# massquantity/LibRecommender

Hardware: AMD Instinct MI355X
Metric: train samples/sec (higher is better)
Workload: dtype f32 (split-bf16 x6 MFMA products, f32 accumulate); 1 GPU; DeepFM ranking train step, 1M users x 1M items x 200 sparse fields (10,000,200 sparse rows), embed_size=64, hidden=(128,64,32), Zipf(1.05) ids; per_gpu_batch=16384, global_batch=16384, fields=202, embed_size=64, table_rows=12000202, parallelism=single, launch=one hipGraph replay per step

## Files before the change

### include/libreco_hip.h

```cpp
#ifndef LIBRECO_HIP_H_
#define LIBRECO_HIP_H_

#include <stddef.h>
#include <stdint.h>

#ifdef __cplusplus
extern "C" {
#endif

#define LR_OK 0
#define LR_EINVAL (-1)
#define LR_ESHAPE (-2)
#define LR_EWORKSPACE (-3)

typedef void* lr_stream_t;

const char* lr_strerror(int code);
int lr_abi_version(void);
int lr_graph_foreign_nodes(void* graph, int* n_nodes_out);

int lr_embed_gather_f32(const float* table, int64_t V, int K, const int32_t* idx,
                        int64_t n, float* out, lr_stream_t stream);

#define LR_COMBINER_SUM 0
// ... 219 lines not shown
int lr_adam_coef_store(lr_adam_hp hp, void* coef_dev, lr_stream_t stream);
int lr_adam_dense_dc_f32(float* table, float* m, float* v, int64_t n, const float* grad,
                         const void* coef_dev, lr_stream_t stream);
int lr_fm_rows_adam_dc_f32(float* table, float* m, float* v, float* lin, float* lin_m, float* lin_v,
                           int64_t V, int K, const float* ge, const float* gl, const float* wp,
                           const float* bn_a, const float* bn_c, const float* lin_scale, int64_t B,
                           int F, const int32_t* seg_pos, const int32_t* seg_rows,
                           const int32_t* seg_start, const int32_t* n_seg, const void* coef_dev,
                           void* ws, size_t ws_bytes, lr_stream_t stream);
int lr_embed_scatter_adam_dc_f32(float* table, float* m, float* v, int64_t V, int K, const float* grad,
                                 const int32_t* seg_pos, const int32_t* seg_rows, const int32_t* seg_start,
                                 const int32_t* n_seg, int64_t n_max, const void* coef_dev,
                                 void* ws, size_t ws_bytes, lr_stream_t stream);
int lr_embed_scatter_adam_lin_dc_f32(float* table, float* m, float* v, int64_t V, int K, const float* grad,
                                     float* lin, float* lin_m, float* lin_v, const float* glin,
                                     const int32_t* seg_pos, const int32_t* seg_rows,
                                     const int32_t* seg_start, const int32_t* n_seg, int64_t n_max,
                                     const void* coef_dev, lr_stream_t stream);

int lr_table_colstats_f32(const float* table, int64_t V, int K, const int32_t* idx, int64_t B, int F, int C,
                          float* partial, lr_stream_t stream);
int lr_bn_remainder_f32(float* G, const float* x, const float* a, const float* c, int64_t rows,
                        int64_t rows_per_plane, int64_t period, int Kp, lr_stream_t stream);

size_t lr_segments_fields_ws_bytes(int64_t B, int F);
int lr_segments_build_fields(const int32_t* idxT, int64_t B, int F, const int32_t* field_row_start,
                             int32_t* seg_pos, int32_t* seg_rows, int32_t* seg_start,
                             int32_t* n_seg, int32_t* slotT, void* ws, size_t ws_bytes,
                             lr_stream_t stream);
int lr_segments_build_fields_runs(const int32_t* idxT, int64_t B, int F, const int32_t* field_row_start,
                                  int32_t* seg_pos, int32_t* seg_rows, int32_t* seg_start,
                                  int32_t* n_seg, int32_t* slotT, int32_t* runT, void* ws, size_t ws_bytes,
                                  lr_stream_t stream);

size_t lr_owner_partition_ws_bytes(int64_t n_max, int W);
int lr_owner_partition_i32(const int32_t* rows, const int32_t* n_seg, int64_t n_max, int W, int32_t* perm,
                           int32_t* send_ids, int64_t* counts, void* ws, size_t ws_bytes, lr_stream_t stream);

size_t lr_din_attn_ws_bytes(int64_t B, int L, int K, int H);
int lr_din_attn_path(int K, int L, int backward);
int lr_din_build_ids_i32(const int32_t* users, const int32_t* items, const int32_t* sparse, int sparse_ld,
                         const int32_t* cols, int n_plain, const int32_t* seqs, const int32_t* lens, int64_t B, int L,
                         int32_t user_off, int32_t item_off, int32_t sparse_off, int32_t* ids, lr_stream_t stream);
int lr_din_attn_pool_fwd_f32(const float* item_table, int64_t V, int K,
                             const int32_t* item, const int32_t* seq, const int32_t* len,
                             int64_t B, int L, const float* W1, const float* b1,
                             const float* W2, const float* b2, int H, float* out,
                             float* attn, float* hid , int32_t* order_out ,
                             lr_stream_t stream);
int lr_din_attn_pool_bwd_f32(const float* item_table, int64_t V, int K,
                             const int32_t* item, const int32_t* seq, const int32_t* len,
                             int64_t B, int L, const float* W1, const float* b1,
                             const float* W2, const float* b2, int H, const float* attn,
                             const float* gout, float* gq, float* gkey, float* gW1,
                             float* gb1, float* gW2, float* gb2, void* ws, size_t ws_bytes,
                             lr_stream_t stream);
int lr_din_attn_pool_bwd_parts_f32(const float* item_table, int64_t V, int K,
                                   const int32_t* item, const int32_t* seq, const int32_t* len,
                                   int64_t B, int L, const float* W1, const float* b1,
                                   const float* W2, const float* b2, int H, const float* attn,
                                   const float* gout, float* gq, float* gkey, float* gW1,
                                   float* gb1, float* gW2, float* gb2, void* ws, size_t ws_bytes,
                                   int parts, int keep_pad_rows, const float* hid ,
                                   const int32_t* order , lr_stream_t stream);
int lr_din_attn_dense_fwd_f32(const float* q, const float* keys, int K, const int32_t* len,
                              int64_t B, int L, const float* W1, const float* b1,
// ... 365 lines not shown
```

### librecommender_amd/_lib.py

```python
from __future__ import annotations

import ctypes as C
import os
from pathlib import Path

LIB_PATH = Path(__file__).resolve().parent / "lib" / "liblibreco_hip.so"

LR_OK, LR_EINVAL, LR_ESHAPE, LR_EWORKSPACE = 0, -1, -2, -3
ABI_VERSION = 26

COMBINERS = {"sum": 0, "mean": 1, "sqrtn": 2}


class AdamHP(C.Structure):

    _fields_ = [
        ("lr", C.c_double),
        ("beta1", C.c_double),
        ("beta2", C.c_double),
        ("eps", C.c_double),
        ("weight_decay", C.c_double),
        ("step", C.c_int32),
        ("tf_style", C.c_int32),
    ]
# ... 102 lines not shown
    "lr_bitmap_ids_i32": (_int, [_p, _i64, _i64, _p, _int, _p]),
    "lr_row_slots_i32": (_int, [_p, _p, _i64, _p, _int, _p]),
    "lr_spmm_csr_adam_f32": (_int, [_p, _p, _p, _i64, _i64, _p, _int, _p, _p, _p, _p, _p, _p, _f32, AdamHP, _p, _sz, _int, _p]),
    "lr_din_build_ids_i32": (_int, [_p, _p, _p, _int, _p, _int, _p, _p, _i64, _int, _int, _int, _int, _p, _p]),
    "lr_softmax_ce_supported": (_int, [_i64, _i64, _int]),
    "lr_softmax_ce_fwd_ws_bytes": (_sz, [_i64, _i64, _int, _int]),
    "lr_softmax_ce_fwd_f32": (_int, [_p, _i64, _p, _i64, _int, _p, _p, _p, _i64, _p, _p, _p, _p, _sz, _int, _p]),
    "lr_softmax_ce_bwd_cols_f32": (_int, [_p, _i64, _p, _i64, _int, _p, _p, _p, _i64, _p, _p, _p, _int, _p]),
    "lr_reduce_job_bytes": (_sz, []),
    "lr_reduce_partials_multi_f32": (_int, [_p, _int, _i64, _p]),
    "lr_pair_mlp_supported": (_int, [_int, _int]),
    "lr_pair_mlp_f32": (_int, [_p, _i64, _p, _i64, _int, _p, _p, _int, _p, _f32, _p, _i64, _int, _p]),
    "lr_pair_mlp_sb_f32": (_int, [_p, _i64, _p, _i64, _int, _p, _p, _int, _p, _f32, _p, _i64, _int, _p]),
    "lr_score_topk_test_mute": (None, [_int]),
    "lr_mfma_f32_probe": (_int, [_int, _int, _p, _p]),
    "lr_probe_occupy": (_int, [_int, _sz, _i64, _p]),
    "lr_clock_probe": (_int, [_p, _p]),
    "lr_clock_probe_slots": (_int, []),
    "lr_mlp_tail3_resident_blocks": (_int, []),
    "lr_adam_coef_bytes": (_sz, []),
    "lr_adam_coef_store": (_int, [AdamHP, _p, _p]),
    "lr_adam_dense_dc_f32": (_int, [_p, _p, _p, _i64, _p, _p, _p]),
    "lr_fm_rows_adam_dc_f32": (_int, [_p, _p, _p, _p, _p, _p, _i64, _int, _p, _p, _p, _p, _p, _p, _i64,
                                      _int, _p, _p, _p, _p, _p, _p, _sz, _p]),
    "lr_embed_scatter_adam_dc_f32": (_int, [_p, _p, _p, _i64, _int, _p, _p, _p, _p, _p, _i64, _p, _p, _sz, _p]),
    "lr_embed_scatter_adam_lin_dc_f32": (_int, [_p, _p, _p, _i64, _int, _p, _p, _p, _p, _p, _p, _p, _p, _p, _i64, _p, _p]),
    "lr_table_colstats_f32": (_int, [_p, _i64, _int, _p, _i64, _int, _int, _p, _p]),
    "lr_bn_remainder_f32": (_int, [_p, _p, _p, _p, _i64, _i64, _i64, _int, _p]),
    "lr_csr_laplacian_ws_bytes": (_sz, [_i64]),
    "lr_csr_laplacian_build": (_int, [_p, _p, _i64, _i64, _i64, _p, _p, _p, _p, _p, _p, _sz, _p]),
    "lr_segments_fields_ws_bytes": (_sz, [_i64, _int]),
    "lr_segments_build_fields": (_int, [_p, _i64, _int, _p, _p, _p, _p, _p, _p, _p, _sz, _p]),
    "lr_segments_build_fields_runs": (_int, [_p, _i64, _int, _p, _p, _p, _p, _p, _p, _p, _p, _sz, _p]),
    "lr_owner_partition_ws_bytes": (_sz, [_i64, _int]),
    "lr_owner_partition_i32": (_int, [_p, _p, _i64, _int, _p, _p, _p, _p, _sz, _p]),
    "lr_din_attn_ws_bytes": (_sz, [_i64, _int, _int, _int]),
    "lr_din_attn_path": (_int, [_int, _int, _int]),
    "lr_din_attn_pool_fwd_f32": (_int, [_p, _i64, _int, _p, _p, _p, _i64, _int, _p, _p, _p, _p,
                                        _int, _p, _p, _p, _p, _p]),
    "lr_din_attn_pool_bwd_f32": (_int, [_p, _i64, _int, _p, _p, _p, _i64, _int, _p, _p, _p, _p,
                                        _int, _p, _p, _p, _p, _p, _p, _p, _p, _p, _sz, _p]),
    "lr_din_attn_pool_bwd_parts_f32": (_int, [_p, _i64, _int, _p, _p, _p, _i64, _int, _p, _p, _p, _p,
                                              _int, _p, _p, _p, _p, _p, _p, _p, _p, _p, _sz, _int, _int, _p, _p, _p]),
    "lr_din_attn_dense_fwd_f32": (_int, [_p, _p, _int, _p, _i64, _int, _p, _p, _p, _p, _int, _p,
                                         _p, _p]),
    "lr_din_attn_dense_bwd_f32": (_int, [_p, _p, _int, _p, _i64, _int, _p, _p, _p, _p, _int, _p,
                                         _p, _p, _p, _p, _p, _p, _p, _p, _sz, _p]),
    "lr_score_topk_ws_bytes": (_sz, [_i64, _i64, _int, _int]),
    "lr_score_topk_f32": (_int, [_p, _i64, _p, _i64, _int, _p, _p, _p, _int, _i64, _p, _p, _p,
                                 _sz, _p]),
    "lr_score_topk_sb_f32": (_int, [_p, _i64, _p, _i64, _int, _p, _p, _p, _int, _i64, _p, _p, _p,
                                 _sz, _p]),
    "lr_score_topk_filter_kp": (_int, [_int]),
    "lr_score_topk_filter_ws_bytes": (_sz, [_i64, _i64, _int, _int]),
    "lr_score_topk_filter_f32": (_int, [_p, _i64, _p, _i64, _int, _p, _p, _p, _int, _i64, _p, _p, _p,
                                        _sz, _int, _int, _p, _p]),
    "lr_topk_merge_f32": (_int, [_p, _p, _int, _i64, _int, _p, _p, _p]),
    "lr_ivf_supported": (_int, [_i64, _i64, _int, _int, _int, _int]),
    "lr_ivf_search_ws_bytes": (_sz, [_i64, _i64, _int, _int, _int, _int]),
    "lr_ivf_build_ws_bytes": (_sz, [_i64, _int]),
    "lr_ivf_centroids_ws_bytes": (_sz, [_i64, _int]),
    "lr_ivf_assign_f32": (_int, [_p, _i64, _p, _int, _int, _p, _p, _p]),
    "lr_ivf_build_lists": (_int, [_p, _i64, _int, _p, _p, _p, _sz, _p]),
    "lr_ivf_centroids_f32": (_int, [_p, _i64, _int, _p, _p, _i64, _int, _p, _p, _sz, _p]),
    "lr_ivf_search_f32": (_int, [_p, _i64, _p, _int, _p, _p, _p, _i64, _int, _p, _p, _p, _int, _int, _p, _p, _p, _sz, _p]),
    "lr_ivf_sq8_supported": (_int, [_i64, _i64, _int, _int, _int, _int, _int]),
# ... 175 lines not shown
```

### librecommender_amd/csrc/segments.hip

```cpp
#include <cstring>

#include <rocprim/rocprim.hpp>

#include "common.hpp"

namespace lr {

__global__ __launch_bounds__(kBlock) void seg_keys_kernel(const int32_t* __restrict__ idx,
                                                          int64_t n, uint32_t V,
                                                          uint32_t* __restrict__ keys) {
  const int64_t stride = static_cast<int64_t>(gridDim.x) * kBlock;
  for (int64_t i = static_cast<int64_t>(blockIdx.x) * kBlock + threadIdx.x; i < n; i += stride) {
    const int32_t id = idx[i];
    keys[i] = (id >= 0 && static_cast<uint32_t>(id) < V) ? static_cast<uint32_t>(id) : V;
  }
}

__global__ __launch_bounds__(kBlock) void seg_heads_kernel(const uint32_t* __restrict__ keys,
                                                           int64_t n, uint32_t V,
                                                           int32_t* __restrict__ heads,
                                                           int32_t* __restrict__ n_seg,
                                                           int32_t* __restrict__ seg_start) {
  const int64_t stride = static_cast<int64_t>(gridDim.x) * kBlock;
  const int64_t t0 = static_cast<int64_t>(blockIdx.x) * kBlock + threadIdx.x;
// ... 150 lines not shown
#pragma unroll
    for (int s = 0; s < kFSE; ++s) x[s] = buf[wid * kFSW + s * 64 + lane];
  }
  if (n_pass == 0) {
#pragma unroll
    for (int s = 0; s < kFSE; ++s) buf[wid * kFSW + s * 64 + lane] = x[s];
  }
  __syncthreads();

  int nv = 0, nh = 0;
  uint64_t* dst = sorted + static_cast<int64_t>(f) * B;
#pragma unroll
  for (int s = 0; s < kFSE; ++s) {
    const int i = wid * kFSW + s * 64 + lane;
    const uint32_t key = static_cast<uint32_t>(x[s] >> 32);
    const bool valid = key != kKeyInvalid;
    const bool head = valid && (i == 0 || static_cast<uint32_t>(buf[i > 0 ? i - 1 : 0] >> 32) != key);
    nv += __popcll(__ballot(valid));
    nh += __popcll(__ballot(head));
    if (i < B) dst[i] = x[s];
  }
  __syncthreads();
  if (lane == 0) { wsum[wid * 2] = nv; wsum[wid * 2 + 1] = nh; }
  __syncthreads();
  if (tid == 0) {
    int tv = 0, th = 0;
    for (int w = 0; w < kSortWaves; ++w) { tv += wsum[2 * w]; th += wsum[2 * w + 1]; }
    fcount[2 * f] = tv;
    fcount[2 * f + 1] = th;
  }
}

constexpr int kEmitThreads = 1024;
constexpr int kEmitWaves = kEmitThreads / 64;

__global__ __launch_bounds__(kEmitThreads) void seg_field_emit_kernel(
    const uint64_t* __restrict__ sorted, const int32_t* __restrict__ fcount, int B, int F,
    const int32_t* __restrict__ frs, int32_t* __restrict__ seg_pos, int32_t* __restrict__ seg_rows,
    int32_t* __restrict__ seg_start, int32_t* __restrict__ n_seg, int32_t* __restrict__ slotT,
    int32_t* __restrict__ runT) {
  __shared__ int red[2][kEmitWaves];
  __shared__ int wh[kEmitWaves];
  const int f = blockIdx.x;
  const int tid = threadIdx.x, wid = tid >> 6, lane = tid & 63;
  const uint64_t lt = (1ull << lane) - 1ull;
  int bv = 0, bh = 0;
  for (int g = tid; g < f; g += kEmitThreads) { bv += fcount[2 * g]; bh += fcount[2 * g + 1]; }
#pragma unroll
  for (int o = 32; o > 0; o >>= 1) { bv += __shfl_xor(bv, o); bh += __shfl_xor(bh, o); }
  if (lane == 0) { red[0][wid] = bv; red[1][wid] = bh; }
  __syncthreads();
  int base_v = 0, base_h = 0;
#pragma unroll
  for (int w = 0; w < kEmitWaves; ++w) { base_v += red[0][w]; base_h += red[1][w]; }
  const int nv = fcount[2 * f];
  const int32_t lo = frs[f];
  const uint64_t* src = sorted + static_cast<int64_t>(f) * B;
  const int chunk = ((B + kEmitWaves - 1) / kEmitWaves + 63) / 64 * 64;
  const int i0 = wid * chunk, i1 = (i0 + chunk) < B ? (i0 + chunk) : B;
  auto is_head = [&](int i, uint32_t key) {
    return i < nv && (i == 0 || static_cast<uint32_t>(src[i - 1] >> 32) != key);
  };
  int heads = 0;
  for (int i = i0 + lane; i < i0 + chunk; i += 64) {
    const bool h = i < i1 && is_head(i, static_cast<uint32_t>(src[i < B ? i : 0] >> 32));
    heads += __popcll(__ballot(h));
  }
  if (lane == 0) wh[wid] = heads;
  __syncthreads();
  int run = base_h;
  for (int w = 0; w < wid; ++w) run += wh[w];
  for (int i = i0 + lane; i < i0 + chunk; i += 64) {
    const bool in = i < i1;
    const uint64_t e = src[in ? i : 0];
    const uint32_t key = static_cast<uint32_t>(e >> 32);
    const int p = static_cast<int>(static_cast<uint32_t>(e));
    const bool h = in && is_head(i, key);
    const uint64_t hb = __ballot(h);
    if (in) {
      const bool valid = i < nv;
      if (valid) seg_pos[base_v + i] = p * F + f;
      if (slotT != nullptr) slotT[static_cast<int64_t>(f) * B + p] = valid ? base_v + i : -1;
      if (runT != nullptr) runT[static_cast<int64_t>(f) * B + p] = valid ? run + __popcll(hb & (lt | (1ull << lane))) - 1 : -1;
      if (h) {
        const int r = run + __popcll(hb & lt);
        seg_rows[r] = lo + static_cast<int32_t>(key);
        seg_start[r] = base_v + i;
      }
    }
    run += __popcll(hb);
  }
  if (f == F - 1 && tid == 0) {
    const int tot_h = base_h + fcount[2 * f + 1];
    seg_start[tot_h] = base_v + nv;
    n_seg[0] = tot_h;
  }
}

constexpr int kRsKPT = 8;
constexpr int kRsKPB = kBlock * kRsKPT;
constexpr int kRsWaves = kBlock / 64;
constexpr int kRsKPW = kRsKPB / kRsWaves;
constexpr int64_t kRsMaxN = int64_t(1) << 22;

__global__ __launch_bounds__(kBlock) void rs_hist_kernel(const uint32_t* __restrict__ keys, int64_t n, int shift, int nblk,
                                                         int32_t* __restrict__ hist) {
  __shared__ int cnt[256];
  const int tid = threadIdx.x;
  cnt[tid] = 0;
  __syncthreads();
  const int64_t base = static_cast<int64_t>(blockIdx.x) * kRsKPB;
#pragma unroll
  for (int st = 0; st < kRsKPT; ++st) {
    const int64_t i = base + st * kBlock + tid;
    if (i < n) atomicAdd(&cnt[(keys[i] >> shift) & 255u], 1);
  }
  __syncthreads();
  hist[static_cast<int64_t>(tid) * nblk + blockIdx.x] = cnt[tid];
}

__global__ __launch_bounds__(64) void rs_scan_kernel(int32_t* __restrict__ hist, int nblk, int32_t* __restrict__ tot) {
  const int d = blockIdx.x, lane = threadIdx.x;
  int32_t* row = hist + static_cast<int64_t>(d) * nblk;
  int carry = 0;
  for (int b0 = 0; b0 < nblk; b0 += 64) {
    const int b = b0 + lane;
    const int v = b < nblk ? row[b] : 0;
    int x = v;
#pragma unroll
    for (int o = 1; o < 64; o <<= 1) {
      const int y = __shfl_up(x, o);
// ... 135 lines not shown
    rocprim::counting_iterator<int32_t> iota(0);
    e = rocprim::radix_sort_pairs(nullptr, need, w.keys_in, w.keys_out, iota, seg_pos, static_cast<size_t>(n), 0u,
                                  static_cast<unsigned>(bits), s);
    if (e != hipSuccess) return static_cast<int>(e);
    if (need > w.prim_bytes) return LR_EWORKSPACE;
    e = rocprim::radix_sort_pairs(w.prim, need, w.keys_in, w.keys_out, iota, seg_pos, static_cast<size_t>(n), 0u,
                                  static_cast<unsigned>(bits), s);
    if (e != hipSuccess) return static_cast<int>(e);
  }

  hipLaunchKernelGGL(seg_heads_kernel, dim3(grid), dim3(kBlock), 0, s, w.keys_out, n, Vu,
                     w.rank, n_seg, seg_start);
  need = 0;
  e = rocprim::inclusive_scan(nullptr, need, w.rank, w.rank, static_cast<size_t>(n),
                              rocprim::plus<int32_t>(), s);
  if (e != hipSuccess) return static_cast<int>(e);
  if (need > w.prim_bytes) return LR_EWORKSPACE;
  e = rocprim::inclusive_scan(w.prim, need, w.rank, w.rank, static_cast<size_t>(n),
                              rocprim::plus<int32_t>(), s);
  if (e != hipSuccess) return static_cast<int>(e);

  hipLaunchKernelGGL(seg_emit_kernel, dim3(grid), dim3(kBlock), 0, s, w.keys_out, w.rank, n,
                     Vu, seg_pos, seg_rows, seg_start, n_seg, pos_to_seg);
  return launch_status();
}

extern "C" size_t lr_segments_fields_ws_bytes(int64_t B, int F) {
  if (B < 0 || F < 1) return 0;
  return align_up(static_cast<size_t>(B) * F * 8) + align_up(static_cast<size_t>(F) * 8);
}

static int build_fields_impl(const int32_t* idxT, int64_t B, int F, const int32_t* field_row_start, int32_t* seg_pos,
                             int32_t* seg_rows, int32_t* seg_start, int32_t* n_seg, int32_t* slotT, int32_t* runT, void* ws,
                             size_t ws_bytes, lr_stream_t stream) {
  LR_CHECK_ARG(B >= 1 && F >= 1);
  LR_CHECK_ARG(idxT && field_row_start && seg_pos && seg_rows && seg_start && n_seg && ws);
  if (B > kFS || B * F >= (int64_t(1) << 31)) return LR_ESHAPE;
  if (ws_bytes < lr_segments_fields_ws_bytes(B, F)) return LR_EWORKSPACE;
  hipStream_t s = as_stream(stream);
  uint64_t* sorted = static_cast<uint64_t*>(ws);
  int32_t* fcount = reinterpret_cast<int32_t*>(static_cast<char*>(ws) + align_up(static_cast<size_t>(B) * F * 8));
  const size_t lds = static_cast<size_t>(kFS) * 8 + kSortWaves * 256 * 4 + kSortWaves * 2 * 4;
  static bool attr_set = false;
  if (!attr_set) {
    hipError_t e = hipFuncSetAttribute(reinterpret_cast<const void*>(seg_field_sort_kernel),
                                       hipFuncAttributeMaxDynamicSharedMemorySize, static_cast<int>(lds));
    if (e != hipSuccess) return static_cast<int>(e);
    attr_set = true;
  }
  hipLaunchKernelGGL(seg_field_sort_kernel, dim3(F), dim3(kSortThreads), lds, s, idxT, static_cast<int>(B),
                     field_row_start, sorted, fcount);
  hipLaunchKernelGGL(seg_field_emit_kernel, dim3(F), dim3(kEmitThreads), 0, s, sorted, fcount,
                     static_cast<int>(B), F, field_row_start, seg_pos, seg_rows, seg_start, n_seg, slotT, runT);
  return launch_status();
}

extern "C" int lr_segments_build_fields(const int32_t* idxT, int64_t B, int F, const int32_t* field_row_start,
                                        int32_t* seg_pos, int32_t* seg_rows, int32_t* seg_start, int32_t* n_seg,
                                        int32_t* slotT, void* ws, size_t ws_bytes, lr_stream_t stream) {
  return build_fields_impl(idxT, B, F, field_row_start, seg_pos, seg_rows, seg_start, n_seg, slotT, nullptr, ws, ws_bytes,
                           stream);
}

extern "C" int lr_segments_build_fields_runs(const int32_t* idxT, int64_t B, int F, const int32_t* field_row_start,
                                             int32_t* seg_pos, int32_t* seg_rows, int32_t* seg_start, int32_t* n_seg,
                                             int32_t* slotT, int32_t* runT, void* ws, size_t ws_bytes, lr_stream_t stream) {
  LR_CHECK_ARG(runT != nullptr);
  return build_fields_impl(idxT, B, F, field_row_start, seg_pos, seg_rows, seg_start, n_seg, slotT, runT, ws, ws_bytes,
                           stream);
}

constexpr int kOwnChunk = 1024;
constexpr int kOwnMaxW = 64;

template <bool kPlace>
__device__ __forceinline__ void owner_chunk(const int32_t* __restrict__ rows, int n, int W, int chunk, int (*cnt)[4][kOwnMaxW],
                                            int* my_owner, int* my_rank) {
  const int tid = threadIdx.x, wid = tid >> 6, lane = tid & 63;
  const uint64_t lt = (1ull << lane) - 1ull;
#pragma unroll
  for (int it = 0; it < 4; ++it) {
    const int i = chunk * kOwnChunk + it * kBlock + tid;
    const int o = i < n ? static_cast<int>(static_cast<uint32_t>(rows[i]) % static_cast<uint32_t>(W)) : -1;
    int rank = 0;
    for (int w = 0; w < W; ++w) {
      const uint64_t mk = __ballot(o == w);
      if (o == w) rank = __popcll(mk & lt);
      if (lane == 0) cnt[it][wid][w] = __popcll(mk);
    }
    if (kPlace) { my_owner[it] = o; my_rank[it] = rank; }
  }
}

__global__ __launch_bounds__(kBlock) void owner_count_kernel(const int32_t* __restrict__ rows, const int32_t* __restrict__ n_seg,
// ... 110 lines not shown
```

### librecommender_amd/layers/dense.py

```python
from __future__ import annotations

import math
import os
from typing import List, Optional, Sequence

import torch
import torch.nn.functional as F

from .. import _lib, ops


class DenseParams:

    def __init__(self, device: torch.device, seed: int = 42):
        self.device = device
        self.gen = torch.Generator(device=device)
        self.gen.manual_seed(seed + 1)
        self._specs = []
        self.params = {}
        self.flat = self.grad = self.m = self.v = None

    def add(self, name: str, shape: Sequence[int], init: str) -> str:
        assert self.flat is None, "finalize() already called"
        self._specs.append((name, tuple(shape), init))
# ... 343 lines not shown
    dgamma = (XhG * W).sum(1)
    dbeta = W @ sgz
    s = gamma * inv
    c = s * inv * (dgamma / B)
    a = s * (dbeta / B) - c * mean
    io.bn_a, io.bn_c = a.contiguous(), c.contiguous()
    return dgamma, dbeta, dW, sgz


class FoldedL1Kernels:

    STAT_CHUNKS = 8

    def __init__(self, P, bn, layer, F: int, K: int, device, stat_chunks: Optional[int] = None):
        self.P, self.bn, self.layer, self.F, self.K, self.device = P, bn, layer, int(F), int(K), device
        n, H1 = self.F * self.K, P[layer.w].shape[1]
        f32 = dict(dtype=torch.float32, device=device)
        self.H1 = H1
        if stat_chunks is not None:
            self.STAT_CHUNKS = int(stat_chunks)
        self.stat_partial = torch.empty((self.F, self.STAT_CHUNKS, 2, self.K), **f32)
        self.mean, self.inv, self.s, self.t = (torch.empty(n, **f32) for _ in range(4))
        self.n_slabs = _lib.load().lr_deepfm_l1_fold_bias_slabs(n)
        self.bias_partial = torch.empty((self.n_slabs, H1), **f32)
        self.bp = torch.empty(H1, **f32)
        self.bn_ac = torch.empty(2 * n, **f32)
        self.bn_a, self.bn_c = self.bn_ac[:n], self.bn_ac[n:]

    @staticmethod
    def supported(H1: int) -> bool:
        return H1 in (64, 128, 256)

    def forward(self, io: "FusedL1IO", seg, field_row_start, B: int, cache_slots: Optional[torch.Tensor] = None,
                sync=None) -> torch.Tensor:
        P, bn, l0, st = self.P, self.bn, self.layer, ops._stream()
        W, b = P[l0.w], P[l0.b]
        n = self.F * self.K
        if bn is not None:
            if seg is None:
                ops.table_colstats(io.table, io.idx, self.STAT_CHUNKS, out=self.stat_partial)
            elif cache_slots is None:
                ops._call("lr_fm_field_stats_f32", ops._ptr(io.table), self.K, ops._ptr(seg.rows), ops._ptr(seg.start),
                          ops._ptr(seg.n_seg), ops._ptr(field_row_start), self.F, self.STAT_CHUNKS, ops._ptr(self.stat_partial), st)
            else:
                ops._call("lr_fm_field_stats_slots_f32", ops._ptr(io.table), self.K, ops._ptr(seg.rows), ops._ptr(seg.start),
                          ops._ptr(seg.n_seg), ops._ptr(field_row_start), self.F, self.STAT_CHUNKS, ops._ptr(self.stat_partial),
                          ops._ptr(seg.pos), ops._ptr(cache_slots), st)
            if sync is not None:
                sync(self.stat_partial)
            if os.environ.get("LIBRECO_FOLD_CHAIN", "merged") == "merged" and self.H1 <= 256 and 256 % self.H1 == 0:
                ops._call("lr_deepfm_l1_fold_stats_bias_f32", ops._ptr(self.stat_partial), self.F, self.STAT_CHUNKS, self.K, B,
                          float(bn.eps), float(bn.momentum), ops._ptr(P[bn.gamma]), ops._ptr(P[bn.beta]),
                          ops._ptr(bn.moving_mean), ops._ptr(bn.moving_var), ops._ptr(self.mean), ops._ptr(self.inv),
                          ops._ptr(self.s), ops._ptr(self.t), ops._ptr(W), ops._ptr(b), self.H1, ops._ptr(self.bias_partial), st)
                WpA, WpB = ops.deepfm_l1_pack(W, self.F, self.K, out=io.pack_bufs, scale=self.s,
                                              reduce=(self.bias_partial, self.bp))
            else:
                ops._call("lr_deepfm_l1_fold_stats_f32", ops._ptr(self.stat_partial), self.F, self.STAT_CHUNKS, self.K, B,
                          float(bn.eps), float(bn.momentum), ops._ptr(P[bn.gamma]), ops._ptr(P[bn.beta]),
                          ops._ptr(bn.moving_mean), ops._ptr(bn.moving_var), ops._ptr(self.mean), ops._ptr(self.inv),
                          ops._ptr(self.s), ops._ptr(self.t), st)
                WpA, WpB = ops.deepfm_l1_pack(W, self.F, self.K, out=io.pack_bufs, scale=self.s)
                ops._call("lr_deepfm_l1_fold_bias_f32", ops._ptr(self.t), ops._ptr(W), ops._ptr(b), n, self.H1,
                          ops._ptr(self.bias_partial), st)
                ops._call("lr_reduce_partials_f32", ops._ptr(self.bias_partial), self.n_slabs, self.H1, self.H1,
                          ops._ptr(self.bp), st)
            bias = self.bp
        else:
            WpA, WpB = ops.deepfm_l1_pack(W, self.F, self.K, out=io.pack_bufs)
            bias = b
        z1, io.pair, io.fsum, io.lin_out = ops.deepfm_l1_fwd(io.table, io.idx, WpA, bias, self.H1, lin=io.lin,
                                                             out=getattr(io, "fwd_bufs", None))
# ... 78 lines not shown
```

### librecommender_amd/nets/fm_nets.py

```python
from __future__ import annotations

from typing import Sequence

import torch

from ..utils.device import to_device
import torch.nn.functional as F

from .. import ops
from ..layers import DenseParams, DenseStack, FieldTables, TFBatchNorm, TFDense
from ..layers.dense import BlockFirstLayer, FoldedL1Kernels, FusedL1IO, fused_l1_backward, fused_l1_forward
from ..layers.tail import DeepFMTail


class _FieldNet:
    def __init__(self, n_users, n_items, sparse_feature_size, n_fields, embed_size, device, seed,
                 lr, epsilon, dense_adam=False, reg=None, tables=None, sparse_offsets=None):
        self.device = device
        self.tables = tables if tables is not None else FieldTables(
            n_users, n_items, sparse_feature_size, embed_size, device, seed, sparse_offsets=sparse_offsets)
        self.F, self.K = int(n_fields), int(embed_size)
        self.P = DenseParams(device, seed)
        self.lr, self.epsilon = lr, epsilon
        self.dense_adam, self.reg = dense_adam, reg or 0.0
# ... 148 lines not shown
            return self._fused_tail(self.mlp.fused_first(io, training=False), io, training=False)
        e, pair, _, lin = ops.fm_embed_fwd(self.tables.embed, idx, lin=self.tables.lin)
        return self._dense_forward(e, pair, lin, training=False, side={})

    def _pack_bufs(self):
        if self._pack is None:
            H1 = self.P[self.mlp.layers[0].w].shape[1]
            self._pack = ops.deepfm_l1_pack_bufs(self.F, self.K, H1, self.device)
        return self._pack

    @property
    def l1_arith(self) -> str:
        return "split_bf16" if self._pack_bufs()[0].dtype == torch.uint8 else "f32_chain"

    def _fused_tail(self, z1, io, training):
        deep = self.mlp.tail(z1, training)
        linear_term = self.linear(io.lin_out)
        concat = torch.cat([linear_term, io.pair, deep], dim=1)
        return self.out(concat).squeeze(1)

    def _fused_core(self, idx, labels, loss_type, hp):
        t, B, F_, K = self.tables, idx.shape[0], self.F, self.K
        dev = self.device
        if self._fseg is None or self._fseg.B_max < B:
            self._graphs = {}
            self._fseg = ops.FieldSegmentBuilder(B, F_, t.V, dev)
            self._idxT = torch.empty((F_, B), dtype=torch.int32, device=dev)
            self._ge = torch.empty((B * F_ + 1, K), dtype=torch.float32, device=dev)
            H1 = self.P[self.mlp.layers[0].w].shape[1]
            nch = ops.deepfm_l1_wgrad_chunks(B, F_, K, H1, self.l1_arith)
            self._wgrad = torch.empty((nch, F_ * K, H1), dtype=torch.float32, device=dev)
        same = B == self._fseg.B_max
        idxT = ops.idx_transpose(idx, out=self._idxT if same else None)
        seg = self._fseg.build(idxT, t.field_row_start)
        io = FusedL1IO(t.embed, t.lin, idx, idxT, F_, K, pack_bufs=self._pack_bufs(),
                       wgrad_buf=self._wgrad if same else None)
        if self.hip_tail and loss_type == "cross_entropy":
            return self._fused_core_hip_tail(io, seg, labels, hp, same)
        stats = ops.fm_field_stats(t.embed, seg, t.field_row_start, B) if self.mlp.bn_in is not None else None
        self.P.zero_grad()
        z1 = self.mlp.fused_first(io, training=True, stats=stats)
        logits = self._fused_tail(z1, io, training=True)
        logits.retain_grad()
        loss = self.loss_fn(logits, labels, loss_type)
        loss.backward()
        with torch.no_grad():
            gl = logits.grad.contiguous()
            w_out = self.P[self.out.w]
            wp = w_out[1:1 + K, 0] + 0.0
            lin_scale = w_out[0, 0] * self.P[self.linear.w][:, 0]
            ge = ops.deepfm_l1_dgrad(io.gz, io.WpB, K, F_, seg.slotT, gl=gl, wp=wp, fsum=io.fsum,
                                     out=self._ge if same else None)
            self._rows_update(ge, seg, hp, B, gl, wp, io, lin_scale, same)
            self.P.adam_step(hp)
        self._last_step = (io, gl, wp, seg)
        return loss.detach()

    @torch.no_grad()
    def _fused_core_hip_tail(self, io, seg, labels, hp, same):
        t, P, mlp = self.tables, self.P, self.mlp
        B, F_, K = io.idx.shape[0], self.F, self.K
        bn, l0 = mlp.bn_in, mlp.layers[0]
        if self._fold is None and FoldedL1Kernels.supported(P[l0.w].shape[1]):
            self._fold = FoldedL1Kernels(P, bn, l0, F_, K, self.device)
        if self._tail is None:
            self._tail = DeepFMTail(P, mlp, self.linear, self.out, F_, K, self.device)
            self._tail.on_release = lambda: setattr(self, "_graphs", {})
        if self._fold is not None:
            z1 = self._fold.forward(io, seg, t.field_row_start, B)
            loss, gl, gz1, sgz1 = self._tail.run(z1, io.pair, io.lin_out, labels)
            self._fold.backward(io, gz1, sgz1)
        else:
            if bn is not None:
                mean, var = ops.fm_field_stats(t.embed, seg, t.field_row_start, B)
                bn.moving_mean.mul_(bn.momentum).add_(mean, alpha=1 - bn.momentum)
                bn.moving_var.mul_(bn.momentum).add_(var, alpha=1 - bn.momentum)
                inv = torch.rsqrt(var + bn.eps)
                gamma, beta = P[bn.gamma], P[bn.beta]
            else:
                mean = inv = gamma = beta = None
            z1 = fused_l1_forward(gamma, beta, P[l0.w], P[l0.b], mean, inv, io)
            loss, gl, gz1, sgz1 = self._tail.run(z1, io.pair, io.lin_out, labels)
            dgamma, dbeta, dW, db = fused_l1_backward(gamma, beta, P[l0.w], mean, inv, io, gz1, sgz1)
            P[l0.w].grad.copy_(dW)
            P[l0.b].grad.copy_(db)
            if bn is not None:
                P[bn.gamma].grad.copy_(dgamma)
                P[bn.beta].grad.copy_(dbeta)
        w_out = P[self.out.w]
        wp = w_out[1:1 + K, 0] + 0.0
        lin_scale = w_out[0, 0] * P[self.linear.w][:, 0]
        ge = ops.deepfm_l1_dgrad(io.gz, io.WpB, K, F_, seg.slotT, gl=gl, wp=wp, fsum=io.fsum,
                                 out=self._ge if same else None)
        self._rows_update(ge, seg, hp, B, gl, wp, io, lin_scale, same)
        P.adam_step(hp)
        self._last_step = (io, gl, wp, seg)
        return loss

    def _rows_update(self, ge, seg, hp, B, gl, wp, io, lin_scale, same):
        t, F_ = self.tables, self.F
        need = ops._lib.load().lr_fm_embed_bwd_ws_bytes(B, F_)
        if self._bwd_ws is None or self._bwd_ws.numel() < need:
# ... 342 lines not shown
```

### librecommender_amd/ops.py

```python
from __future__ import annotations

import os

from dataclasses import dataclass
from typing import NamedTuple, Optional

import torch

from . import _lib
from ._lib import AdamHP, COMBINERS, check


def _stream() -> int:
    return torch.cuda.current_stream().cuda_stream


class KernelTimer:

    def __init__(self):
        self.names = set()
        self.events = {}

    def enable(self, *names):
        self.names = set(names)
# ... 170 lines not shown
        n = idx.numel()
        if n > self.n_max:
            raise ValueError(f"idx has {n} entries, builder was sized for {self.n_max}")
        if want_slots and self.slots is None:
            self.slots = torch.empty(self.n_max, dtype=torch.int32, device=self.device)
        _call("lr_segments_build", _ptr(idx), n, self.V, _ptr(self.pos), _ptr(self.rows),
                                            _ptr(self.start), _ptr(self.n_seg),
                                            _ptr(self.slots) if want_slots else None, _ptr(self.ws),
                                            self.ws.numel(), _stream())
        seg = Segments(self.pos, self.rows, self.start, self.n_seg, n, self.V, owner=self)
        seg.slots = self.slots[:n] if want_slots else None
        return seg


def build_segments(idx: torch.Tensor, V: int) -> Segments:
    return SegmentBuilder(max(idx.numel(), 1), V, idx.device).build(idx)


class FieldSegmentBuilder:

    MAX_B = 16384

    def __init__(self, B_max: int, F: int, V: int, device: torch.device, want_runs: bool = False):
        self.B_max, self.F, self.V, self.device = int(B_max), int(F), int(V), device
        n = self.B_max * self.F
        self.ws = torch.empty(_lib.load().lr_segments_fields_ws_bytes(self.B_max, self.F), dtype=torch.uint8, device=device)
        self.pos = torch.empty(n, dtype=torch.int32, device=device)
        self.rows = torch.empty(n, dtype=torch.int32, device=device)
        self.start = torch.empty(n + 1, dtype=torch.int32, device=device)
        self.n_seg = torch.zeros(1, dtype=torch.int32, device=device)
        self.slotT = torch.empty((self.F, self.B_max), dtype=torch.int32, device=device)
        self.runT = torch.empty((self.F, self.B_max), dtype=torch.int32, device=device) if want_runs else None

    def build(self, idxT: torch.Tensor, field_row_start: torch.Tensor) -> Segments:
        _req(idxT, torch.int32, "idxT", 2)
        _req(field_row_start, torch.int32, "field_row_start", 1)
        F, B = idxT.shape
        if F != self.F or B > self.B_max or field_row_start.numel() != F + 1:
            raise ValueError("idxT does not match this builder")
        cut = (lambda t: t if B == self.B_max else t.view(-1)[: F * B].view(F, B))
        slotT = cut(self.slotT)
        seg = Segments(self.pos, self.rows, self.start, self.n_seg, B * F, self.V)
        if self.runT is None:
            _call("lr_segments_build_fields", _ptr(idxT), B, F, _ptr(field_row_start), _ptr(self.pos), _ptr(self.rows),
                  _ptr(self.start), _ptr(self.n_seg), _ptr(slotT), _ptr(self.ws), self.ws.numel(), _stream())
        else:
            seg.runT = cut(self.runT)
            _call("lr_segments_build_fields_runs", _ptr(idxT), B, F, _ptr(field_row_start), _ptr(self.pos), _ptr(self.rows),
                  _ptr(self.start), _ptr(self.n_seg), _ptr(slotT), _ptr(seg.runT), _ptr(self.ws), self.ws.numel(), _stream())
        seg.slotT = slotT
        return seg


class OwnerPartition:

    def __init__(self, n_max: int, W: int, device: torch.device):
        self.n_max, self.W = int(n_max), int(W)
        self.ws = torch.empty(max(_lib.load().lr_owner_partition_ws_bytes(self.n_max, self.W), 256), dtype=torch.uint8, device=device)
        self.perm = torch.empty(self.n_max, dtype=torch.int32, device=device)
        self.send_ids = torch.empty(self.n_max, dtype=torch.int32, device=device)
        self.counts = torch.zeros(self.W + 1, dtype=torch.int64, device=device)

    def run(self, rows: torch.Tensor, n_seg: torch.Tensor):
        _req(rows, torch.int32, "rows", 1)
        _req(n_seg, torch.int32, "n_seg", 1)
        if rows.numel() > self.n_max:
            raise ValueError("rows exceed this partition's capacity")
        _call("lr_owner_partition_i32", _ptr(rows), _ptr(n_seg), rows.numel(), self.W, _ptr(self.perm), _ptr(self.send_ids),
              _ptr(self.counts), _ptr(self.ws), self.ws.numel(), _stream())
        return self.perm, self.send_ids, self.counts


def idx_transpose(idx: torch.Tensor, out: Optional[torch.Tensor] = None) -> torch.Tensor:
    _req(idx, torch.int32, "idx", 2)
    B, F = idx.shape
    if out is None:
# ... 2957 lines not shown
```

Baseline: 6.460 million samples/s.

## Fuse batch-norm field column stats into segment emit kernel launch

Adds a combined kernel that runs the per-field segment emit blocks and extra per-(field, chunk) blocks computing BN input column sums and squared sums. The stats blocks read the already sorted keys and load each distinct embedding row once, weighting it by its run length. This replaces the separate field-stats kernel in the fused DeepFM tail path, saving a launch and a pass over the indices. In exchange, emit blocks drop from 1024 to 512 threads, and the stats blocks share a grid with emit work, which may change occupancy and balance.

```diff
diff --git a/include/libreco_hip.h b/include/libreco_hip.h
--- a/include/libreco_hip.h
+++ b/include/libreco_hip.h
@@ -275,6 +275,10 @@
                                   int32_t* seg_pos, int32_t* seg_rows, int32_t* seg_start,
                                   int32_t* n_seg, int32_t* slotT, int32_t* runT, void* ws, size_t ws_bytes,
                                   lr_stream_t stream);
+int lr_segments_build_fields_stats_f32(const int32_t* idxT, int64_t B, int F, const int32_t* field_row_start,
+                                       int32_t* seg_pos, int32_t* seg_rows, int32_t* seg_start, int32_t* n_seg,
+                                       int32_t* slotT, void* ws, size_t ws_bytes, const float* table, int K, int C,
+                                       float* partial, lr_stream_t stream);
 
 size_t lr_owner_partition_ws_bytes(int64_t n_max, int W);
 int lr_owner_partition_i32(const int32_t* rows, const int32_t* n_seg, int64_t n_max, int W, int32_t* perm,
diff --git a/librecommender_amd/_lib.py b/librecommender_amd/_lib.py
--- a/librecommender_amd/_lib.py
+++ b/librecommender_amd/_lib.py
@@ -158,6 +158,7 @@
     "lr_segments_fields_ws_bytes": (_sz, [_i64, _int]),
     "lr_segments_build_fields": (_int, [_p, _i64, _int, _p, _p, _p, _p, _p, _p, _p, _sz, _p]),
     "lr_segments_build_fields_runs": (_int, [_p, _i64, _int, _p, _p, _p, _p, _p, _p, _p, _p, _sz, _p]),
+    "lr_segments_build_fields_stats_f32": (_int, [_p, _i64, _int, _p, _p, _p, _p, _p, _p, _p, _sz, _p, _int, _int, _p, _p]),
     "lr_owner_partition_ws_bytes": (_sz, [_i64, _int]),
     "lr_owner_partition_i32": (_int, [_p, _p, _i64, _int, _p, _p, _p, _p, _sz, _p]),
     "lr_din_attn_ws_bytes": (_sz, [_i64, _int, _int, _int]),
diff --git a/librecommender_amd/csrc/segments.hip b/librecommender_amd/csrc/segments.hip
--- a/librecommender_amd/csrc/segments.hip
+++ b/librecommender_amd/csrc/segments.hip
@@ -206,31 +206,31 @@
 }
 
 constexpr int kEmitThreads = 1024;
-constexpr int kEmitWaves = kEmitThreads / 64;
-
-__global__ __launch_bounds__(kEmitThreads) void seg_field_emit_kernel(
-    const uint64_t* __restrict__ sorted, const int32_t* __restrict__ fcount, int B, int F,
+
+template <int kThreads>
+__device__ __forceinline__ void seg_field_emit_body(
+    const int f, const uint64_t* __restrict__ sorted, const int32_t* __restrict__ fcount, int B, int F,
     const int32_t* __restrict__ frs, int32_t* __restrict__ seg_pos, int32_t* __restrict__ seg_rows,
     int32_t* __restrict__ seg_start, int32_t* __restrict__ n_seg, int32_t* __restrict__ slotT,
     int32_t* __restrict__ runT) {
-  __shared__ int red[2][kEmitWaves];
-  __shared__ int wh[kEmitWaves];
-  const int f = blockIdx.x;
+  constexpr int kWaves = kThreads / 64;
+  __shared__ int red[2][kWaves];
+  __shared__ int wh[kWaves];
   const int tid = threadIdx.x, wid = tid >> 6, lane = tid & 63;
   const uint64_t lt = (1ull << lane) - 1ull;
   int bv = 0, bh = 0;
-  for (int g = tid; g < f; g += kEmitThreads) { bv += fcount[2 * g]; bh += fcount[2 * g + 1]; }
+  for (int g = tid; g < f; g += kThreads) { bv += fcount[2 * g]; bh += fcount[2 * g + 1]; }
 #pragma unroll
   for (int o = 32; o > 0; o >>= 1) { bv += __shfl_xor(bv, o); bh += __shfl_xor(bh, o); }
   if (lane == 0) { red[0][wid] = bv; red[1][wid] = bh; }
   __syncthreads();
   int base_v = 0, base_h = 0;
 #pragma unroll
-  for (int w = 0; w < kEmitWaves; ++w) { base_v += red[0][w]; base_h += red[1][w]; }
+  for (int w = 0; w < kWaves; ++w) { base_v += red[0][w]; base_h += red[1][w]; }
   const int nv = fcount[2 * f];
   const int32_t lo = frs[f];
   const uint64_t* src = sorted + static_cast<int64_t>(f) * B;
-  const int chunk = ((B + kEmitWaves - 1) / kEmitWaves + 63) / 64 * 64;
+  const int chunk = ((B + kWaves - 1) / kWaves + 63) / 64 * 64;
   const int i0 = wid * chunk, i1 = (i0 + chunk) < B ? (i0 + chunk) : B;
   auto is_head = [&](int i, uint32_t key) {
     return i < nv && (i == 0 || static_cast<uint32_t>(src[i - 1] >> 32) != key);
@@ -271,6 +271,125 @@
   }
 }
 
+__global__ __launch_bounds__(kEmitThreads) void seg_field_emit_kernel(
+    const uint64_t* __restrict__ sorted, const int32_t* __restrict__ fcount, int B, int F,
+    const int32_t* __restrict__ frs, int32_t* __restrict__ seg_pos, int32_t* __restrict__ seg_rows,
+    int32_t* __restrict__ seg_start, int32_t* __restrict__ n_seg, int32_t* __restrict__ slotT,
+    int32_t* __restrict__ runT) {
+  seg_field_emit_body<kEmitThreads>(blockIdx.x, sorted, fcount, B, F, frs, seg_pos, seg_rows, seg_start, n_seg, slotT, runT);
+}
+
+constexpr int kFusedThreads = 512;
+constexpr int kFusedWaves = kFusedThreads / 64;
+constexpr int kFusedWavesPerSimd = 6;
+
+template <int LPR>
+__device__ __forceinline__ void field_stats_sorted(const int f, const int c, const int C,
+                                                   const uint64_t* __restrict__ sorted,
+                                                   const int32_t* __restrict__ fcount, int B,
+                                                   const int32_t* __restrict__ frs, const float* __restrict__ table,
+                                                   float* __restrict__ partial) {
+  constexpr int K = LPR * 4, NG = kFusedThreads / LPR;
+  __shared__ double fold[kFusedWaves][2][4][LPR];
+  const int tid = threadIdx.x, wid = tid >> 6, lane = tid & 63;
+  const int gl = lane % LPR, gbase = lane - gl, grp = tid / LPR;
+  const int nv = fcount[2 * f];
+  const int beg = static_cast<int>(static_cast<int64_t>(nv) * c / C);
+  const int len = static_cast<int>(static_cast<int64_t>(nv) * (c + 1) / C) - beg;
+  const int g0 = beg + static_cast<int>(static_cast<int64_t>(len) * grp / NG);
+  const int g1 = beg + static_cast<int>(static_cast<int64_t>(len) * (grp + 1) / NG);
+  const int nb = ((len + NG - 1) / NG + LPR - 1) / LPR;
+  const uint64_t* src = sorted + static_cast<int64_t>(f) * B;
+  const float* rows = table + static_cast<int64_t>(frs[f]) * K + gl * 4;
+  auto batch_key = [&](int b) -> uint32_t {
+    const int i = g0 + b * LPR + gl;
+    return i < g1 ? static_cast<uint32_t>(src[i] >> 32) : kKeyInvalid;
+  };
+  double ds[4] = {0.0, 0.0, 0.0, 0.0}, dq[4] = {0.0, 0.0, 0.0, 0.0};
+  uint32_t nxt = nb > 0 ? batch_key(0) : kKeyInvalid;
+  for (int b = 0; b < nb; ++b) {
+    const uint32_t id = nxt;
+    if (b + 1 < nb) nxt = batch_key(b + 1);
+    const int left_n = g1 - (g0 + b * LPR);
+    const int nvalid = left_n < 0 ? 0 : (left_n < LPR ? left_n : LPR);
+    const uint32_t left = __shfl_up(id, 1);
+    const bool head = gl < nvalid && (gl == 0 || id != left);
+    uint32_t m = static_cast<uint32_t>((__ballot(head) >> gbase) & ((1ull << LPR) - 1ull));
+    while (__ballot(m != 0u) != 0ull) {
+      float cn[4];
+      float4 w[4];
+#pragma unroll
+      for (int j = 0; j < 4; ++j) {
+        const bool v = m != 0u;
+        const int h = v ? __ffs(static_cast<int>(m)) - 1 : 0;
+        m &= m - 1u;
+        const int nh = m != 0u ? __ffs(static_cast<int>(m)) - 1 : nvalid;
+        cn[j] = v ? static_cast<float>(nh - h) : 0.f;
+        const uint32_t rid = __shfl(id, gbase + h);
+        w[j] = v ? ld4(rows + static_cast<int64_t>(rid) * K) : f4_zero();
+      }
+#pragma unroll
+      for (int j = 0; j < 4; ++j) {
+        const double cd = cn[j];
+        const double x[4] = {w[j].x, w[j].y, w[j].z, w[j].w};
+#pragma unroll
+        for (int i = 0; i < 4; ++i) {
+          const double cx = cd * x[i];
+          ds[i] += cx;
+          dq[i] = fma(cx, x[i], dq[i]);
+        }
+      }
+    }
+  }
+#pragma unroll
+  for (int o = LPR; o < 64; o <<= 1) {
+#pragma unroll
+    for (int j = 0; j < 4; ++j) {
+      ds[j] += __shfl_xor(ds[j], o);
+      dq[j] += __shfl_xor(dq[j], o);
+    }
+  }
+  if (lane < LPR) {
+#pragma unroll
+    for (int j = 0; j < 4; ++j) {
+      fold[wid][0][j][gl] = ds[j];
+      fold[wid][1][j][gl] = dq[j];
+    }
+  }
+  __syncthreads();
+  if (tid < LPR) {
+    double ts[4] = {0.0, 0.0, 0.0, 0.0}, tq[4] = {0.0, 0.0, 0.0, 0.0};
+#pragma unroll 4
+    for (int w = 0; w < kFusedWaves; ++w) {
+#pragma unroll
+      for (int j = 0; j < 4; ++j) {
+        ts[j] += fold[w][0][j][gl];
+        tq[j] += fold[w][1][j][gl];
+      }
+    }
+    float* dst = partial + (static_cast<int64_t>(f) * C + c) * 2 * K;
+    st4(dst + gl * 4, make_float4(static_cast<float>(ts[0]), static_cast<float>(ts[1]), static_cast<float>(ts[2]),
+                                  static_cast<float>(ts[3])));
+    st4(dst + K + gl * 4, make_float4(static_cast<float>(tq[0]), static_cast<float>(tq[1]), static_cast<float>(tq[2]),
+                                      static_cast<float>(tq[3])));
+  }
+}
+
+template <int LPR>
+__global__ __launch_bounds__(kFusedThreads, kFusedWavesPerSimd) void seg_field_emit_stats_kernel(
+    const uint64_t* __restrict__ sorted, const int32_t* __restrict__ fcount, int B, int F,
+    const int32_t* __restrict__ frs, int32_t* __restrict__ seg_pos, int32_t* __restrict__ seg_rows,
+    int32_t* __restrict__ seg_start, int32_t* __restrict__ n_seg, int32_t* __restrict__ slotT,
+    const float* __restrict__ table, int C, float* __restrict__ partial) {
+  const int blk = blockIdx.x;
+  if (blk < F) {
+    seg_field_emit_body<kFusedThreads>(blk, sorted, fcount, B, F, frs, seg_pos, seg_rows, seg_start, n_seg, slotT, nullptr);
+  } else {
+    const int u = blk - F;
+    field_stats_sorted<LPR>(u / C, u % C, C, sorted, fcount, B, frs, table, partial);
+  }
+}
+
 constexpr int kRsKPT = 8;
 constexpr int kRsKPB = kBlock * kRsKPT;
 constexpr int kRsWaves = kBlock / 64;
@@ -472,10 +591,16 @@
 
 static int build_fields_impl(const int32_t* idxT, int64_t B, int F, const int32_t* field_row_start, int32_t* seg_pos,
                              int32_t* seg_rows, int32_t* seg_start, int32_t* n_seg, int32_t* slotT, int32_t* runT, void* ws,
-                             size_t ws_bytes, lr_stream_t stream) {
+                             size_t ws_bytes, lr_stream_t stream, const float* table = nullptr, int K = 0, int C = 0,
+                             float* partial = nullptr) {
   LR_CHECK_ARG(B >= 1 && F >= 1);
   LR_CHECK_ARG(idxT && field_row_start && seg_pos && seg_rows && seg_start && n_seg && ws);
   if (B > kFS || B * F >= (int64_t(1) << 31)) return LR_ESHAPE;
+  if (table != nullptr) {
+    LR_CHECK_ARG(partial && C >= 1 && runT == nullptr);
+    LR_CHECK_ARG(reinterpret_cast<uintptr_t>(table) % 16 == 0 && reinterpret_cast<uintptr_t>(partial) % 16 == 0);
+    if ((K != 16 && K != 32 && K != 64 && K != 128) || static_cast<int64_t>(F) * (C + 1) >= (int64_t(1) << 31)) return LR_ESHAPE;
+  }
   if (ws_bytes < lr_segments_fields_ws_bytes(B, F)) return LR_EWORKSPACE;
   hipStream_t s = as_stream(stream);
   uint64_t* sorted = static_cast<uint64_t*>(ws);
@@ -490,8 +615,19 @@
   }
   hipLaunchKernelGGL(seg_field_sort_kernel, dim3(F), dim3(kSortThreads), lds, s, idxT, static_cast<int>(B),
                      field_row_start, sorted, fcount);
-  hipLaunchKernelGGL(seg_field_emit_kernel, dim3(F), dim3(kEmitThreads), 0, s, sorted, fcount,
-                     static_cast<int>(B), F, field_row_start, seg_pos, seg_rows, seg_start, n_seg, slotT, runT);
+  if (table == nullptr) {
+    hipLaunchKernelGGL(seg_field_emit_kernel, dim3(F), dim3(kEmitThreads), 0, s, sorted, fcount,
+                       static_cast<int>(B), F, field_row_start, seg_pos, seg_rows, seg_start, n_seg, slotT, runT);
+    return launch_status();
+  }
+#define LR_FES(LPR)                                                                                              \
+  hipLaunchKernelGGL((seg_field_emit_stats_kernel<LPR>), dim3(F + F * C), dim3(kFusedThreads), 0, s, sorted, fcount, \
+                     static_cast<int>(B), F, field_row_start, seg_pos, seg_rows, seg_start, n_seg, slotT, table, C, partial)
+  if (K == 16) LR_FES(4);
+  else if (K == 32) LR_FES(8);
+  else if (K == 64) LR_FES(16);
+  else LR_FES(32);
+#undef LR_FES
   return launch_status();
 }
 
@@ -500,6 +636,15 @@
                                         int32_t* slotT, void* ws, size_t ws_bytes, lr_stream_t stream) {
   return build_fields_impl(idxT, B, F, field_row_start, seg_pos, seg_rows, seg_start, n_seg, slotT, nullptr, ws, ws_bytes,
                            stream);
+}
+
+extern "C" int lr_segments_build_fields_stats_f32(const int32_t* idxT, int64_t B, int F, const int32_t* field_row_start,
+                                                  int32_t* seg_pos, int32_t* seg_rows, int32_t* seg_start, int32_t* n_seg,
+                                                  int32_t* slotT, void* ws, size_t ws_bytes, const float* table, int K, int C,
+                                                  float* partial, lr_stream_t stream) {
+  LR_CHECK_ARG(table != nullptr);
+  return build_fields_impl(idxT, B, F, field_row_start, seg_pos, seg_rows, seg_start, n_seg, slotT, nullptr, ws, ws_bytes,
+                           stream, table, K, C, partial);
 }
 
 extern "C" int lr_segments_build_fields_runs(const int32_t* idxT, int64_t B, int F, const int32_t* field_row_start,
diff --git a/librecommender_amd/layers/dense.py b/librecommender_amd/layers/dense.py
--- a/librecommender_amd/layers/dense.py
+++ b/librecommender_amd/layers/dense.py
@@ -399,12 +399,14 @@
         return H1 in (64, 128, 256)
 
     def forward(self, io: "FusedL1IO", seg, field_row_start, B: int, cache_slots: Optional[torch.Tensor] = None,
-                sync=None) -> torch.Tensor:
+                sync=None, stats_ready: bool = False) -> torch.Tensor:
         P, bn, l0, st = self.P, self.bn, self.layer, ops._stream()
         W, b = P[l0.w], P[l0.b]
         n = self.F * self.K
         if bn is not None:
-            if seg is None:
+            if stats_ready:
+                pass
+            elif seg is None:
                 ops.table_colstats(io.table, io.idx, self.STAT_CHUNKS, out=self.stat_partial)
             elif cache_slots is None:
                 ops._call("lr_fm_field_stats_f32", ops._ptr(io.table), self.K, ops._ptr(seg.rows), ops._ptr(seg.start),
diff --git a/librecommender_amd/nets/fm_nets.py b/librecommender_amd/nets/fm_nets.py
--- a/librecommender_amd/nets/fm_nets.py
+++ b/librecommender_amd/nets/fm_nets.py
@@ -204,11 +204,14 @@
             self._wgrad = torch.empty((nch, F_ * K, H1), dtype=torch.float32, device=dev)
         same = B == self._fseg.B_max
         idxT = ops.idx_transpose(idx, out=self._idxT if same else None)
-        seg = self._fseg.build(idxT, t.field_row_start)
+        hip_tail = self.hip_tail and loss_type == "cross_entropy"
+        fold = self._fold_kernels() if hip_tail else None
+        stats = (t.embed, fold.stat_partial) if fold is not None and fold.bn is not None else None
+        seg = self._fseg.build(idxT, t.field_row_start, stats=stats)
         io = FusedL1IO(t.embed, t.lin, idx, idxT, F_, K, pack_bufs=self._pack_bufs(),
                        wgrad_buf=self._wgrad if same else None)
-        if self.hip_tail and loss_type == "cross_entropy":
-            return self._fused_core_hip_tail(io, seg, labels, hp, same)
+        if hip_tail:
+            return self._fused_core_hip_tail(io, seg, labels, hp, same, stats_ready=stats is not None)
         stats = ops.fm_field_stats(t.embed, seg, t.field_row_start, B) if self.mlp.bn_in is not None else None
         self.P.zero_grad()
         z1 = self.mlp.fused_first(io, training=True, stats=stats)
@@ -228,18 +231,23 @@
         self._last_step = (io, gl, wp, seg)
         return loss.detach()
 
+    def _fold_kernels(self):
+        l0 = self.mlp.layers[0]
+        if self._fold is None and FoldedL1Kernels.supported(self.P[l0.w].shape[1]):
+            self._fold = FoldedL1Kernels(self.P, self.mlp.bn_in, l0, self.F, self.K, self.device)
+        return self._fold
+
     @torch.no_grad()
-    def _fused_core_hip_tail(self, io, seg, labels, hp, same):
+    def _fused_core_hip_tail(self, io, seg, labels, hp, same, stats_ready=False):
         t, P, mlp = self.tables, self.P, self.mlp
         B, F_, K = io.idx.shape[0], self.F, self.K
         bn, l0 = mlp.bn_in, mlp.layers[0]
-        if self._fold is None and FoldedL1Kernels.supported(P[l0.w].shape[1]):
-            self._fold = FoldedL1Kernels(P, bn, l0, F_, K, self.device)
+        self._fold_kernels()
         if self._tail is None:
             self._tail = DeepFMTail(P, mlp, self.linear, self.out, F_, K, self.device)
             self._tail.on_release = lambda: setattr(self, "_graphs", {})
         if self._fold is not None:
-            z1 = self._fold.forward(io, seg, t.field_row_start, B)
+            z1 = self._fold.forward(io, seg, t.field_row_start, B, stats_ready=stats_ready)
             loss, gl, gz1, sgz1 = self._tail.run(z1, io.pair, io.lin_out, labels)
             self._fold.backward(io, gz1, sgz1)
         else:
diff --git a/librecommender_amd/ops.py b/librecommender_amd/ops.py
--- a/librecommender_amd/ops.py
+++ b/librecommender_amd/ops.py
@@ -226,7 +226,7 @@
         self.slotT = torch.empty((self.F, self.B_max), dtype=torch.int32, device=device)
         self.runT = torch.empty((self.F, self.B_max), dtype=torch.int32, device=device) if want_runs else None
 
-    def build(self, idxT: torch.Tensor, field_row_start: torch.Tensor) -> Segments:
+    def build(self, idxT: torch.Tensor, field_row_start: torch.Tensor, stats=None) -> Segments:
         _req(idxT, torch.int32, "idxT", 2)
         _req(field_row_start, torch.int32, "field_row_start", 1)
         F, B = idxT.shape
@@ -235,7 +235,17 @@
         cut = (lambda t: t if B == self.B_max else t.view(-1)[: F * B].view(F, B))
         slotT = cut(self.slotT)
         seg = Segments(self.pos, self.rows, self.start, self.n_seg, B * F, self.V)
-        if self.runT is None:
+        if stats is not None:
+            table, partial = stats
+            _req(table, torch.float32, "table", 2)
+            _req(partial, torch.float32, "partial", 4)
+            K = table.shape[1]
+            if self.runT is not None or partial.shape[0] != F or tuple(partial.shape[2:]) != (2, K):
+                raise ValueError("stats need a builder without runs and partial [F, C, 2, K]")
+            _call("lr_segments_build_fields_stats_f32", _ptr(idxT), B, F, _ptr(field_row_start), _ptr(self.pos),
+                  _ptr(self.rows), _ptr(self.start), _ptr(self.n_seg), _ptr(slotT), _ptr(self.ws), self.ws.numel(),
+                  _ptr(table), K, int(partial.shape[1]), _ptr(partial), _stream())
+        elif self.runT is None:
             _call("lr_segments_build_fields", _ptr(idxT), B, F, _ptr(field_row_start), _ptr(self.pos), _ptr(self.rows),
                   _ptr(self.start), _ptr(self.n_seg), _ptr(slotT), _ptr(self.ws), self.ws.numel(), _stream())
         else:
```

Measured after the change: 6.502 million samples/s, median of 3. About the same (+0.7%).
